# yjhuangcd/FI-ODE

Hardware: AMD Instinct MI355X
Metric: CIFAR-10 train-step images/sec (B=128, h_sample=256) at 1/2/4/8 MI355X (higher is better)
Workload: dtype f32; 1 GPU; hipGraph replay: BASELINE configs[1]: train step of README.md:27 at epoch 20 with train_ode (rk4, step_size 0.1, t_max=1: 10 steps / 40 train-mode f-evals, backprop through the stages; loss_ode portion 0.2) + the Lyapunov loss (B=128, h_sample_size=256 -> 204 uniform + 52 correct-cone rows/image), KWLarge-Cayley backbone + Adam; global_batch=128, h_sample_size=256, rows_per_rank=32768, parallelism=dp1

## Files before the change

fi-ode_amd/csrc/dense.hip:

```cpp
#include <hip/hip_runtime.h>
#include <stdint.h>

#include "common.h"
#include "fiode.h"

namespace {

constexpr int NT = 256;
constexpr int DPARTS = 256;

struct DArgs {
  int cout, cin, k, R, wide;
  const float* W;
  const float* alpha;
  const float* nrm;
};

__device__ __forceinline__ float wx(const DArgs& a, const float* Wb, int r, int c) {
  return a.wide ? Wb[(int64_t)c * a.cin + r] : Wb[(int64_t)r * a.cin + c];
}
__device__ __forceinline__ int64_t wpos(const DArgs& a, int r, int c) {
  return a.wide ? (int64_t)c * a.cin + r : (int64_t)r * a.cin + c;
}

// ... 134 lines not shown
  const float s = a.alpha[b] / a.nrm[b];
  const float* Wb = a.W + (int64_t)b * n;
  const float* P1b = P1 ? P1 + (int64_t)b * RV * k : nullptr;
  const float* P2b = P2 ? P2 + (int64_t)b * RV * k : nullptr;
  float* gXb = gX + (int64_t)b * n;
  float d = 0.f;
#pragma unroll 4
  for (int idx = blockIdx.x * NT + threadIdx.x; idx < n; idx += DPARTS * NT) {
    const int o = idx / a.cin, c = idx % a.cin;
    const int r = a.wide ? c : o;
    float g;
    if (r < k) {
      g = gXb[idx];
    } else {
      const int64_t pi = a.wide ? (int64_t)o * RV + (c - k) : (int64_t)(o - k) * k + c;
      g = s * P1b[pi] - 2.0f * P2b[pi];
      gXb[idx] = g;
    }
    d = fmaf(g, Wb[idx], d);
  }
  for (int o = 32; o > 0; o >>= 1) d += __shfl_xor(d, o);
  if ((threadIdx.x & 63) == 0) red[threadIdx.x >> 6] = d;
  __syncthreads();
  if (threadIdx.x == 0) {
    float t = 0.f;
    for (int q = 0; q < NT / 64; ++q) t += red[q];
    dpart[b * DPARTS + blockIdx.x] = t;
  }
}

__global__ void __launch_bounds__(NT) k_dense_gv4(DArgs a, const float* __restrict__ P1, const float* __restrict__ P2,
// ... 4 lines not shown
  const float* Wb = a.W + (int64_t)b * n;
  const float* P1b = P1 ? P1 + (int64_t)b * RV * k : nullptr;
  const float* P2b = P2 ? P2 + (int64_t)b * RV * k : nullptr;
  float* gXb = gX + (int64_t)b * n;
  float d = 0.f;
  for (int o = blockIdx.x; o < a.cout; o += DPARTS) {
    for (int c4 = threadIdx.x; c4 < c4n; c4 += NT) {
      const int c = 4 * c4;
      const int r = a.wide ? c : o;
      const int64_t idx = (int64_t)o * a.cin + c;
      f32x4 g;
      if (r < k) {
        g = *reinterpret_cast<const f32x4*>(gXb + idx);
      } else {
        const int64_t pi = a.wide ? (int64_t)o * RV + (c - k) : (int64_t)(o - k) * k + c;
        const f32x4 p1 = *reinterpret_cast<const f32x4*>(P1b + pi), p2 = *reinterpret_cast<const f32x4*>(P2b + pi);
#pragma unroll
        for (int e = 0; e < 4; ++e) g[e] = s * p1[e] - 2.0f * p2[e];
        *reinterpret_cast<f32x4*>(gXb + idx) = g;
      }
      const f32x4 w = *reinterpret_cast<const f32x4*>(Wb + idx);
#pragma unroll
      for (int e = 0; e < 4; ++e) d = fmaf(g[e], w[e], d);
    }
  }
  for (int o = 32; o > 0; o >>= 1) d += __shfl_xor(d, o);
  if ((threadIdx.x & 63) == 0) red[threadIdx.x >> 6] = d;
  __syncthreads();
  if (threadIdx.x == 0) {
    float t = 0.f;
    for (int q = 0; q < NT / 64; ++q) t += red[q];
    dpart[b * DPARTS + blockIdx.x] = t;
  }
// ... 78 lines not shown
      for (int x = 0; x < 2; ++x)
#pragma unroll
        for (int y = 0; y < 2; ++y)
          acc[x][y] = __builtin_amdgcn_mfma_f32_16x16x4f32(av[x][s], bv[y][s], acc[x][y], 0, 0, 0);
  }
#pragma unroll
  for (int x = 0; x < 2; ++x)
#pragma unroll
    for (int y = 0; y < 2; ++y)
#pragma unroll
      for (int r = 0; r < 4; ++r) red[w][16 * x + 4 * q + r][16 * y + i] = acc[x][y][r];
  __syncthreads();
  for (int e = threadIdx.x; e < 32 * 32; e += 256) {
    const int r = e >> 5, c = e & 31;
    C[(int64_t)(tm + r) * n + tn + c] = ((red[0][r][c] + red[1][r][c]) + red[2][r][c]) + red[3][r][c];
  }
}

int mk(const fiode_dense_config* cfg, DArgs& a, int& batch) {
  if (!cfg || cfg->batch < 1 || cfg->cout < 1 || cfg->cin < 1) return FIODE_EINVAL;
  a = DArgs{};
  a.cout = cfg->cout;
  a.cin = cfg->cin;
  a.wide = a.cin > a.cout;
  a.k = a.wide ? a.cout : a.cin;
  a.R = a.wide ? a.cin : a.cout;
  batch = cfg->batch;
  return FIODE_OK;
}

// ... 131 lines not shown
  a.nrm = nrm;
  hipStream_t st = (hipStream_t)stream;
  float* dpart = (float*)workspace;
  auto al16 = [](const void* q) { return ((uintptr_t)q & 15u) == 0; };
  const bool vec = a.cin % 4 == 0 && a.k % 4 == 0 && al16(W) && al16(gX) && al16(gW) && (!P1 || al16(P1)) &&
                   (!P2 || al16(P2));
  if (vec)
    hipLaunchKernelGGL(k_dense_gv4, dim3(DPARTS, batch), dim3(NT), 0, st, a, P1, P2, gX, dpart);
  else
    hipLaunchKernelGGL(k_dense_gv, dim3(DPARTS, batch), dim3(NT), 0, st, a, P1, P2, gX, dpart);
  hipLaunchKernelGGL(k_dense_gw, grid_for((int64_t)a.cout * a.cin, batch), dim3(NT), 0, st, a, (const float*)gX, dpart,
                     gW, galpha, vec ? 1 : 0);
  DENSE_RET();
}

extern "C" int fiode_dense_gemm(void* stream, int32_t batch, int32_t n, int32_t trans_a, int32_t trans_b,
                                const float* A, const float* B, float* C) {
  if (batch < 1 || batch > 65535 || n < 64 || !A || !B || !C) return FIODE_EINVAL;
  if (n % 64 != 0) return FIODE_ESHAPE;
  if ((((uintptr_t)A | (uintptr_t)B) & 15u) != 0) return FIODE_ESHAPE;
  const dim3 grid((unsigned)(n / 32), (unsigned)(n / 32), (unsigned)batch);
  hipStream_t st = (hipStream_t)stream;
  if (trans_a && trans_b) hipLaunchKernelGGL((k_dense_gemm<true, true>), grid, dim3(256), 0, st, n, A, B, C);
  else if (trans_a) hipLaunchKernelGGL((k_dense_gemm<true, false>), grid, dim3(256), 0, st, n, A, B, C);
  else if (trans_b) hipLaunchKernelGGL((k_dense_gemm<false, true>), grid, dim3(256), 0, st, n, A, B, C);
  else hipLaunchKernelGGL((k_dense_gemm<false, false>), grid, dim3(256), 0, st, n, A, B, C);
  DENSE_RET();
}
```

fi-ode_amd/fiode_amd/_lib.py:

```python
from __future__ import annotations

import ctypes as ct
import os
import pathlib

_HERE = pathlib.Path(__file__).resolve().parent
LIB_PATH = pathlib.Path(os.environ.get("FIODE_LIB", _HERE / "libfiode.so"))

FIODE_SAMPLER_GIVEN, FIODE_SAMPLER_COMPOSITE, FIODE_SAMPLER_DECISION_BOUNDARY, FIODE_SAMPLER_TRAJECTORY = 0, 1, 2, 3
FIODE_DROPOUT_OFF, FIODE_DROPOUT_GIVEN, FIODE_DROPOUT_PHILOX = 0, 1, 2
FIODE_ACT_RELU, FIODE_ACT_GROUPSORT = 0, 1

class FiodeLibraryError(RuntimeError):
    pass


class FiodeError(RuntimeError):
    pass


_fp = ct.POINTER(ct.c_float)
_vp = ct.c_void_p


# ... 171 lines not shown
        "fiode_dense_cayley_prep": (ct.c_int, [_vp, ct.POINTER(DenseConfig), _vp, _vp, _vp, _vp, _vp]),
        "fiode_dense_norm_workspace_bytes": (ct.c_size_t, [ct.POINTER(DenseConfig)]),
        "fiode_dense_norm_partials": (ct.c_int, [_vp, ct.POINTER(DenseConfig), _vp, _vp, ct.c_size_t]),
        "fiode_dense_cayley_prep_normed": (ct.c_int, [_vp, ct.POINTER(DenseConfig), _vp, _vp, _vp, _vp, _vp, _vp]),
        "fiode_dense_norm_partials_clear": (ct.c_int, [_vp, ct.POINTER(DenseConfig), _vp, _vp, ct.c_size_t, _vp,
                                                       ct.c_size_t, ct.c_size_t]),
        "fiode_dense_inverse_flag_bytes": (ct.c_size_t, [ct.c_int32]),
        "fiode_dense_cayley_inverse": (ct.c_int, [_vp, ct.POINTER(DenseConfig), _vp, _vp, _vp, _vp, _vp, _vp, _vp,
                                                  _vp, ct.c_size_t]),
        "fiode_dense_cayley_finish": (ct.c_int, [_vp, ct.POINTER(DenseConfig), _vp, _vp, _vp, _vp, _vp]),
        "fiode_dense_cayley_ginv": (ct.c_int, [_vp, ct.POINTER(DenseConfig), _vp, _vp, _vp, _vp, _vp]),
        "fiode_dense_cayley_h": (ct.c_int, [_vp, ct.POINTER(DenseConfig), _vp, _vp, _vp]),
        "fiode_dense_cayley_workspace_bytes": (ct.c_size_t, [ct.POINTER(DenseConfig)]),
        "fiode_dense_cayley_grad": (ct.c_int, [_vp, ct.POINTER(DenseConfig), _vp, _vp, _vp, _vp, _vp, _vp, _vp, _vp,
                                               _vp, ct.c_size_t]),
        "fiode_dense_gemm": (ct.c_int, [_vp, ct.c_int32, ct.c_int32, ct.c_int32, ct.c_int32, _vp, _vp, _vp]),
        "fiode_gemm_splits": (ct.c_int32, [ct.POINTER(GemmDesc)]),
        "fiode_gemm_counter_bytes": (ct.c_size_t, [ct.POINTER(GemmDesc)]),
        "fiode_gemm_workspace_bytes": (ct.c_size_t, [ct.POINTER(GemmDesc)]),
        "fiode_gemm": (ct.c_int, [_vp, ct.POINTER(GemmDesc), _vp, _vp, _vp, _vp, _vp, ct.c_size_t]),
        "fiode_gemm_pair_workspace_bytes": (ct.c_size_t, [ct.POINTER(GemmDesc), ct.POINTER(GemmDesc)]),
        "fiode_gemm_pair": (ct.c_int, [_vp, ct.POINTER(GemmDesc), _vp, _vp, _vp, _vp, ct.POINTER(GemmDesc), _vp, _vp,
                                       _vp, _vp, _vp, ct.c_size_t]),
        "fiode_sconv_rfft2": (ct.c_int, [_vp, ct.POINTER(SconvConfig), _vp, _vp, _vp, _vp]),
        "fiode_sconv_irfft2": (ct.c_int, [_vp, ct.POINTER(SconvConfig), _vp, _vp, ct.c_int32, _vp, _vp]),
        "fiode_sconv_rfft2_nchw": (ct.c_int, [_vp, ct.POINTER(SconvConfig), _vp, _vp, _vp, _vp]),
        "fiode_sconv_irfft2_qx": (ct.c_int, [_vp, ct.POINTER(SconvConfig), _vp, _vp, ct.c_int32, _vp, ct.c_int32,
                                             _vp, _vp]),
        "fiode_cgemm": (ct.c_int, [_vp, ct.c_int32, ct.c_int32, ct.c_int32, ct.c_int32, ct.c_int32, ct.c_int32, _vp,
                                   _vp, _vp, _vp]),
# ... 40 lines not shown
```

fi-ode_amd/fiode_amd/cayley.py:

```python
from __future__ import annotations

import ctypes as ct
import math
from typing import Optional

import torch
import torch.nn as nn
import torch.nn.functional as F

from .streams import current, fork, join, prefetch, run_on, shared, take


_BLOCK = 128


def _block_inverse(M: torch.Tensor) -> torch.Tensor:
    from . import ops
    n = M.shape[-1]
    if n > 64 and M.dtype == torch.float32 and M.is_cuda:
        if M.dim() == 2:
            return ops.block_inverse(M)
        return ops.block_inverse(M.reshape(-1, n, n)).reshape(M.shape)
    if n <= _BLOCK:
        return ops.batched_inverse(M)
# ... 172 lines not shown
                     device=Wb.device)
    L.check(lib.fiode_dense_cayley_grad(st, ct.byref(cfg), Wb.data_ptr(), al.data_ptr(), nrm.data_ptr(),
                                        ops._ptr(P1), ops._ptr(P2), gX.data_ptr(), gW.data_ptr(), ga.data_ptr(),
                                        ws.data_ptr(), ws.numel()), "fiode_dense_cayley_grad")
    return gW.reshape(wshape), ga.reshape(ashape)


def _dense_fused_ok(W: torch.Tensor) -> bool:
    from . import _lib as L
    k = min(W.shape[-2], W.shape[-1])
    lib = L.lib()
    return (DENSE_FUSED_INVERSE and W.is_cuda and hasattr(lib, "fiode_dense_cayley_inverse")
            and lib.fiode_dense_inverse_flag_bytes(k) > 0)


def _dense_forward_fused(W: torch.Tensor, alpha: torch.Tensor):
    from . import ops, _lib as L
    Wb = W.detach().reshape(-1, W.shape[-2], W.shape[-1]).contiguous()
    al = alpha.detach().reshape(-1).contiguous().float()
    b, cout, cin = Wb.shape
    wide = cin > cout
    k = cout if wide else cin
    cfg = L.DenseConfig(b, cout, cin)
    lib, stream = L.lib(), ops._stream(W.device)
    per = lib.fiode_block_inverse_workspace_bytes(k)
    ws = ops._Workspace.get(W.device, b * per, f"denseinv{torch.cuda.current_stream(W.device).cuda_stream}")
    part = torch.empty(lib.fiode_dense_norm_workspace_bytes(ct.byref(cfg)) // 4, dtype=torch.float32, device=W.device)
    L.check(lib.fiode_dense_norm_partials_clear(stream, ct.byref(cfg), Wb.data_ptr(), part.data_ptr(), part.numel() * 4,
                                                ws.data_ptr(), lib.fiode_dense_inverse_flag_bytes(k) // 4, per),
            "fiode_dense_norm_partials_clear")
    Vp = (Wb[:, :, k:].mT if wide else Wb[:, k:, :]) if max(cout, cin) > k else None
    G = ops.mm(Vp.mT, Vp, site="dense_fwd") if Vp is not None else None
    nrm = torch.empty(b, dtype=torch.float32, device=W.device)
    inv = torch.empty((b, k, k), dtype=torch.float32, device=W.device)
    Q = torch.empty_like(Wb) if Vp is None else None
    L.check(lib.fiode_dense_cayley_inverse(stream, ct.byref(cfg), Wb.data_ptr(), al.data_ptr(), part.data_ptr(),
                                           ops._ptr(G), nrm.data_ptr(), inv.data_ptr(), ops._ptr(Q), ws.data_ptr(),
                                           ws.numel()), "fiode_dense_cayley_inverse")
    st = dict(Wb=Wb, al=al, nrm=nrm, wide=wide, k=k, Vp=Vp, cfg=cfg)
    if Q is None:
        Q = _dense_finish(st, inv)
    return st, inv, Q


class _DenseCayleyFn(torch.autograd.Function):

    @staticmethod
    def forward(ctx, W, alpha):
        if _dense_fused_ok(W):
            st, inv, Q = _dense_forward_fused(W, alpha)
        else:
            st, M = _dense_prep(W, alpha)
            inv = _block_inverse(M)
            Q = _dense_finish(st, inv)
        ctx.save_for_backward(st["Wb"], st["al"], st["nrm"], inv)
# ... 78 lines not shown
        return top
    return torch.cat([top, -2.0 * (V @ inv)], dim=-2)


DENSE_GEMM = True
DENSE_NORM_PARTIALS = True


class CayleyLinear(nn.Linear):

    def __init__(self, in_features: int, out_features: int, bias: bool = True):
        super().__init__(in_features, out_features, bias)
        self.alpha = nn.Parameter(self.weight.detach().norm().reshape(1).clone())
        self._Q = None
        self._pre = None

    def reset_parameters(self) -> None:
        std = 1.0 / math.sqrt(self.weight.shape[1])
        nn.init.uniform_(self.weight, -std, std)
        if self.bias is not None:
            nn.init.uniform_(self.bias, -std, std)
        self._Q = None

    def effective_weight(self) -> torch.Tensor:
        return cayley_scaled(self.weight, self.alpha)

    def prefetch(self, stream: torch.cuda.Stream) -> None:
        self._pre = prefetch(stream, self.effective_weight)

    def forward_weight_unjoined(self):
        if self._pre is not None and self.training:
            (Q, ev), self._pre = self._pre, None
            Q.record_stream(torch.cuda.current_stream(Q.device))
            self._Q = Q.detach()
            return Q, ev
        return self.forward_weight(), None

    def forward_weight(self) -> torch.Tensor:
        if self._pre is not None and self.training:
            Q = take(self._pre)
            self._pre = None
        elif self.training or self._Q is None:
            Q = self.effective_weight()
        else:
            Q = self._Q
        self._Q = Q.detach()
        return Q if self.training else self._Q

    def forward(self, x: torch.Tensor) -> torch.Tensor:
        return F.linear(x, self.forward_weight(), self.bias)


HEAD_WGRAD_SIDE = True
# ... 31 lines not shown
        g = g.contiguous()

        def wgrad(k, gk, x):
            return fork(_head_stream(g.device, k), lambda: (ops.mm(gk.t(), x, site="head"), gk.sum(0)), reads=(gk, x))

        w3 = wgrad(3, g, z2)
        g2 = ops.head_out_backward_gs(g, Q3, y2) if ctx.out_k else ops.groupsort_backward(y2, ops.mm(g, Q3, site="head"), 1)
        w2 = wgrad(2, g2, z1)
        g1 = ops.groupsort_backward(y1, ops.mm(g2, Q2, site="head"), 1)
        w1 = wgrad(1, g1, h)
        dh = ops.mm(g1, Q1, site="head")
        (dW3, db3), (dW2, db2), (dW1, db1) = join(w3, w2, w1)
        return dh, dW1, db1, dW2, db2, dW3, db3, None


HEAD_OUT_KERNEL = True
HEAD_OUT_MAX_J = 16


def _head_out_ok(Q3: torch.Tensor) -> bool:
    return HEAD_OUT_KERNEL and Q3.shape[0] <= HEAD_OUT_MAX_J


def linear_head(mods, h: torch.Tensor):
    fusable = (HEAD_WGRAD_SIDE and h.is_cuda and len(mods) == 5 and
               all(isinstance(m, CayleyLinear) and m.training and m.bias is not None for m in mods[0::2]) and
               all(isinstance(m, GroupSort) for m in mods[1::2]) and torch.is_grad_enabled())
    if not fusable:
        for m in mods:
            h = m(h)
        return h
    l1, l2, l3 = mods[0::2]
    Q1 = l1.forward_weight()
    (Q2, j2), (Q3, j3) = l2.forward_weight_unjoined(), l3.forward_weight_unjoined()
    return _LinearHeadFn.apply(h.contiguous(), Q1, l1.bias, Q2, l2.bias, Q3, l3.bias, (j2, j3))


class _GroupSortFn(torch.autograd.Function):
    @staticmethod
    def forward(ctx, x, cdim: int):
        from . import ops
        y = ops.groupsort_forward(x, cdim)
        ctx.save_for_backward(x)
        ctx.cdim = cdim
        return y

    @staticmethod
# ... 263 lines not shown
```

fi-ode_amd/fiode_amd/checkpoint.py:

```python
from __future__ import annotations

import os
from typing import Any, Dict, Iterable, Optional, Tuple

import torch
from torch import nn

LIGHTNING_VERSION = "1.6.0"


class CheckpointError(RuntimeError):
    pass


def read_checkpoint(path: str | os.PathLike, map_location: Any = "cpu") -> Dict[str, Any]:
    try:
        ck = torch.load(path, map_location=map_location, weights_only=True)
    except Exception as e:
        raise CheckpointError(f"cannot read {path} with torch.load(weights_only=True): {e}") from e
    if not isinstance(ck, dict):
        raise CheckpointError(f"{path}: expected a dict checkpoint, got {type(ck).__name__}")
    return ck


# ... 4 lines not shown
        raise CheckpointError(f"non-tensor entries in the state_dict: {bad[:5]}")
    return sd


def load_state(module: nn.Module, state_dict: Dict[str, torch.Tensor], strict: bool = False
               ) -> Tuple[list, list]:
    own = module.state_dict()
    shape_bad = [(k, tuple(v.shape), tuple(own[k].shape)) for k, v in state_dict.items()
                 if k in own and tuple(own[k].shape) != tuple(v.shape)]
    if shape_bad:
        raise CheckpointError("shape mismatch (key, checkpoint, module): " + "; ".join(map(str, shape_bad[:5])))
    res = module.load_state_dict(state_dict, strict=strict)
    for m in module.modules():
        if getattr(m, "_pre", None) is not None:
            m._pre = None
    return list(res.missing_keys), list(res.unexpected_keys)


def load_from_checkpoint(module: nn.Module, path: str | os.PathLike, strict: bool = False,
                         map_location: Any = None) -> Dict[str, Any]:
    ck = read_checkpoint(path, map_location="cpu" if map_location is None else map_location)
    sd = checkpoint_state_dict(ck)
    missing, unexpected = load_state(module, sd, strict=strict)
    return dict(missing_keys=missing, unexpected_keys=unexpected, epoch=ck.get("epoch"),
                global_step=ck.get("global_step"))


def save_checkpoint(module: nn.Module, path: str | os.PathLike, epoch: int = 0, global_step: int = 0,
                    optimizers: Optional[Iterable[torch.optim.Optimizer]] = None,
                    extra: Optional[Dict[str, Any]] = None) -> None:
# ... 40 lines not shown
```

fi-ode_amd/fiode_amd/models.py:

```python
from __future__ import annotations

from typing import Optional, Sequence

import torch
import torch.nn as nn

from .cayley import CayleyConv, CayleyLinear, GroupSort, linear_head


class Normalize(nn.Module):

    def __init__(self, mu: Sequence[float], std: Optional[Sequence[float]]):
        super().__init__()
        self.register_buffer("mu", torch.tensor(list(mu), dtype=torch.float32).view(-1, 1, 1))
        self.register_buffer("std", None if std is None else torch.tensor(list(std), dtype=torch.float32).view(-1, 1, 1))

    fused_hwcb = True

    def forward(self, x):
        if self.fused_hwcb and x.is_cuda and x.dtype == torch.float32 and x.dim() == 4 and not x.requires_grad:
            from . import _lib as L, ops
            B, C, H, W = x.shape
            xc = x.contiguous()
            y = torch.empty((H, W, C, B), dtype=torch.float32, device=x.device)
# ... 15 lines not shown
        act_fn = GroupSort if act == "GroupSort" else nn.ReLU
        self.model = nn.Sequential(
            CayleyConv(3, 32 * w, 3), act_fn(),
            CayleyConv(32 * w, 32 * w, 3, stride=2), act_fn(),
            CayleyConv(32 * w, 64 * w, 3), act_fn(),
            CayleyConv(64 * w, 64 * w, 3, stride=2), act_fn(),
            nn.Flatten(),
            CayleyLinear(4096 * w, 512 * w), act_fn(),
            CayleyLinear(512 * w, 512), act_fn(),
            CayleyLinear(512, out_dim),
        )

        self.spatial_major = True
        self.fused_transforms = True
        self.nchw_last = True

    def can_take_nchw(self, x) -> bool:
        m = self.model[0]
        return (self.spatial_major and self.fused_transforms and x.is_cuda and x.dtype == torch.float32
                and x.dim() == 4 and not x.requires_grad and isinstance(m, CayleyConv) and not m.downsample
                and x.shape[-1] == x.shape[-2] and x.shape[-1] in (8, 16, 32))

    def forward(self, x, norm=None):
        if not (self.spatial_major and x.is_cuda):
            return self.model(x)
        mods = list(self.model)
        i = 0
        nconv = 0
        if norm is not None:
            if getattr(self, "after_conv_hook", None) is not None:
                self.after_conv_hook(-1)
            gs = isinstance(mods[1], GroupSort)
            h = mods[0].forward_nchw_fused(x, norm[0], norm[1], gs)
            i = 2 if gs else 1
            if getattr(self, "after_conv_hook", None) is not None:
                self.after_conv_hook(0)
            nconv = 1
        else:
            h = x.permute(2, 3, 1, 0).contiguous()
            if getattr(self, "after_conv_hook", None) is not None:
                self.after_conv_hook(-1)
# ... 8 lines not shown
                    i += 2 if gs else 1
                    if getattr(self, "after_conv_hook", None) is not None:
                        self.after_conv_hook(nconv)
                    nconv += 1
                    continue
                h = m.forward_hwcb(h)
                if getattr(self, "after_conv_hook", None) is not None:
                    self.after_conv_hook(nconv)
                nconv += 1
            elif isinstance(m, GroupSort):
                h = m(h, channel_dim=2)
            else:
                h = m(h)
            i += 1
        h = h.reshape(h.shape[0], -1) if nchw else h.permute(3, 2, 0, 1).reshape(h.shape[3], -1)
        return linear_head(mods[i + 1:], h)


class NormalizedBackbone(nn.Sequential):

    fused_input = True

    def forward(self, x):
        norm, net = self[0], self[1]
        if (self.fused_input and len(self) == 2 and isinstance(norm, Normalize) and isinstance(net, KWLargeConcat)
                and norm.fused_hwcb and net.can_take_nchw(x)):
            return net(x.contiguous(), norm=(norm.mu, norm.std))
        return super().forward(x)


def make_ortho_KWLarge_Concat(n_in_channels=3, n_outputs=10, mu=(0.485, 0.456, 0.406), std=(0.225, 0.225, 0.225),
# ... 47 lines not shown
```

fi-ode_amd/fiode_amd/ops.py:

```python
from __future__ import annotations

import ctypes as ct
from dataclasses import dataclass
from typing import Dict, Optional

import torch

from . import _lib as L

C, M, X = 10, 128, 10
WEIGHT_KEYS = ("Q1", "b1", "Qx", "bx", "Q2", "b2", "Q3", "b3")
WEIGHT_SHAPES = {"Q1": (M, C), "b1": (M,), "Qx": (M, X), "bx": (M,), "Q2": (M, M), "b2": (M,),
                 "Q3": (C, M), "b3": (C,)}


@dataclass
class DynCfg:
    alpha_1: float = 100.0
    alpha_2: float = 20.0
    sigma_1: float = 0.02
    scale_nominal: bool = True
    dropout: float = 0.5
    qp_max_iter: int = 30
    qp_tol: float = 1e-4
# ... 690 lines not shown
                                _ptr(scale), A.data_ptr(), B.data_ptr(), C.data_ptr()), "fiode_cgemm")
    return C


def _mat_layout(X: torch.Tensor):
    R, Cn = X.shape[-2], X.shape[-1]
    s0, s1 = X.stride(-2), X.stride(-1)
    if (s1 == 1 or Cn == 1) and (s0 >= Cn or R == 1):
        return 0, max(s0 if R > 1 else Cn, Cn, 1)
    if (s0 == 1 or R == 1) and (s1 >= R or Cn == 1):
        return 1, max(s1 if Cn > 1 else R, R, 1)
    return None


MM_LIBRARY = False
MM_LIBRARY_SITES: set = {"dense_fwd", "dense_bwd", "head"}
MM_PAIR = True


def _gemm_ws(dev: torch.device, nbytes: int) -> torch.Tensor:
    return _Workspace.get(dev, nbytes, f"gemm{torch.cuda.current_stream(dev).cuda_stream}", zero=True)


def _gemm_operands(A: torch.Tensor, B: torch.Tensor, alpha: float, beta: float, bias, out, split_k: int,
                   max_workgroups: int):
    dev = B.device
    if A.dtype != torch.float32 or B.dtype != torch.float32 or A.device != dev or dev.type != "cuda":
        raise ValueError(f"mm: float32 ROCm operands, got {A.dtype} on {A.device}, {B.dtype} on {B.device}")
    if A.dim() not in (2, 3) or B.dim() not in (2, 3) or A.shape[-1] != B.shape[-2]:
        raise ValueError(f"mm: shapes {tuple(A.shape)} @ {tuple(B.shape)}")
    batch = max(A.shape[0] if A.dim() == 3 else 1, B.shape[0] if B.dim() == 3 else 1)
# ... 27 lines not shown
                   float(alpha), float(beta), int(split_k), int(max_workgroups))
    return d, A, B, bias, out


def mm(A: torch.Tensor, B: torch.Tensor, *, alpha: float = 1.0, beta: float = 0.0,
       bias: Optional[torch.Tensor] = None, out: Optional[torch.Tensor] = None, split_k: int = 0,
       max_workgroups: int = 0, site: str = "") -> torch.Tensor:
    dev = B.device
    if MM_LIBRARY or site in MM_LIBRARY_SITES:
        if out is None and alpha == 1.0 and beta == 0.0:
            if bias is not None and A.dim() == 2 and B.dim() == 2:
                return torch.addmm(bias, A, B)
            r = torch.matmul(A, B)
            return (r + bias if bias is not None else r).contiguous()
        d, A, B, bias, out = _gemm_operands(A, B, alpha, beta, bias, out, split_k, max_workgroups)
        r = torch.matmul(A, B)
        r = r * alpha if alpha != 1.0 else r
        if bias is not None:
            r = r + bias
        if beta != 0.0:
            r = r + beta * out
        out.copy_(r)
        return out
    d, A, B, bias, out = _gemm_operands(A, B, alpha, beta, bias, out, split_k, max_workgroups)
    lib = L.lib()
    nb = lib.fiode_gemm_workspace_bytes(ct.byref(d))
    ws = _gemm_ws(dev, nb) if nb else None
    L.check(lib.fiode_gemm(_stream(dev), ct.byref(d), A.data_ptr(), B.data_ptr(), _ptr(bias), out.data_ptr(),
                           _ptr(ws), ws.numel() if ws is not None else 0), "fiode_gemm")
    return out
# ... 134 lines not shown
```

include/fiode.h:

```cpp
#ifndef FIODE_H_
#define FIODE_H_

#include <stddef.h>
#include <stdint.h>

#ifdef __cplusplus
extern "C" {
#endif

#define FIODE_ABI_VERSION 5

#if defined(__GNUC__)
#define FIODE_API __attribute__((visibility("default")))
#else
#define FIODE_API
#endif

enum {
  FIODE_OK = 0,
  FIODE_EINVAL = 1,
  FIODE_ESHAPE = 2,
  FIODE_EWORKSPACE = 3,
  FIODE_EHIP = 100
};
// ... 241 lines not shown
                                              void* workspace, size_t workspace_bytes, void* clear,
                                              size_t clear_words, size_t clear_stride_bytes);
FIODE_API size_t fiode_dense_inverse_flag_bytes(int32_t k);
FIODE_API int fiode_dense_cayley_inverse(void* stream, const fiode_dense_config* cfg, const float* W,
                                         const float* alpha, const float* part, const float* G, float* nrm_out,
                                         float* inv_out, float* q_out, void* workspace, size_t workspace_bytes);
FIODE_API int fiode_dense_cayley_finish(void* stream, const fiode_dense_config* cfg, const float* alpha,
                                        const float* nrm, const float* inv, const float* P, float* Q);
FIODE_API int fiode_dense_cayley_ginv(void* stream, const fiode_dense_config* cfg, const float* alpha,
                                      const float* nrm, const float* gQ, const float* A, float* Ginv);
FIODE_API int fiode_dense_cayley_h(void* stream, const fiode_dense_config* cfg, const float* GMn, float* gX, float* H);
FIODE_API size_t fiode_dense_cayley_workspace_bytes(const fiode_dense_config* cfg);
FIODE_API int fiode_dense_cayley_grad(void* stream, const fiode_dense_config* cfg, const float* W, const float* alpha,
                                      const float* nrm, const float* P1, const float* P2, float* gX, float* gW,
                                      float* galpha, void* workspace, size_t workspace_bytes);
FIODE_API int fiode_dense_gemm(void* stream, int32_t batch, int32_t n, int32_t trans_a, int32_t trans_b,
                               const float* A, const float* B, float* C);

typedef struct fiode_gemm_desc {
  int32_t batch, M, N, K;
  int32_t trans_a, trans_b;
  int64_t lda, ldb, ldc;
  int64_t stride_a, stride_b, stride_c;
  float alpha, beta;
  int32_t split_k;
  int32_t max_workgroups;
} fiode_gemm_desc;
FIODE_API int32_t fiode_gemm_splits(const fiode_gemm_desc* d);
FIODE_API size_t fiode_gemm_counter_bytes(const fiode_gemm_desc* d);
FIODE_API size_t fiode_gemm_workspace_bytes(const fiode_gemm_desc* d);
// ... 75 lines not shown
```

Baseline: 106,400 images/s.

## Apply first Cayley head layer in factored form instead of materializing Q

For the wide first linear layer of the head, the Cayley-orthogonal weight Q is no longer built explicitly. The head applies the inverse directly to the batch (h minus scaled T, times inv) using new skinny MFMA kernels, with matching input-grad and symmetric pair kernels for the backward pass and a merged weight-gradient path. This skips the O(k^2·cin) finish GEMM and its backward, in exchange for extra per-batch GEMMs, new autograd plumbing and side-stream joins. It also routes plain 2D library matmuls straight to torch.mm/addmm.

```diff
diff --git a/fi-ode_amd/csrc/dense.hip b/fi-ode_amd/csrc/dense.hip
--- a/fi-ode_amd/csrc/dense.hip
+++ b/fi-ode_amd/csrc/dense.hip
@@ -172,7 +172,7 @@
       g = gXb[idx];
     } else {
       const int64_t pi = a.wide ? (int64_t)o * RV + (c - k) : (int64_t)(o - k) * k + c;
-      g = s * P1b[pi] - 2.0f * P2b[pi];
+      g = P2b ? s * P1b[pi] - 2.0f * P2b[pi] : P1b[pi];
       gXb[idx] = g;
     }
     d = fmaf(g, Wb[idx], d);
@@ -207,9 +207,14 @@
         g = *reinterpret_cast<const f32x4*>(gXb + idx);
       } else {
         const int64_t pi = a.wide ? (int64_t)o * RV + (c - k) : (int64_t)(o - k) * k + c;
-        const f32x4 p1 = *reinterpret_cast<const f32x4*>(P1b + pi), p2 = *reinterpret_cast<const f32x4*>(P2b + pi);
-#pragma unroll
-        for (int e = 0; e < 4; ++e) g[e] = s * p1[e] - 2.0f * p2[e];
+        const f32x4 p1 = *reinterpret_cast<const f32x4*>(P1b + pi);
+        if (P2b) {
+          const f32x4 p2 = *reinterpret_cast<const f32x4*>(P2b + pi);
+#pragma unroll
+          for (int e = 0; e < 4; ++e) g[e] = s * p1[e] - 2.0f * p2[e];
+        } else {
+          g = p1;
+        }
         *reinterpret_cast<f32x4*>(gXb + idx) = g;
       }
       const f32x4 w = *reinterpret_cast<const f32x4*>(Wb + idx);
@@ -318,6 +323,169 @@
   for (int e = threadIdx.x; e < 32 * 32; e += 256) {
     const int r = e >> 5, c = e & 31;
     C[(int64_t)(tm + r) * n + tn + c] = ((red[0][r][c] + red[1][r][c]) + red[2][r][c]) + red[3][r][c];
+  }
+}
+
+template <int NW, int UNR, class LA, class LB>
+__device__ __forceinline__ void skinny_wave(int K, int w, int q, LA load_a, LB load_b, f32x4 (&acc)[2][2]) {
+#pragma unroll
+  for (int x = 0; x < 2; ++x)
+#pragma unroll
+    for (int y = 0; y < 2; ++y) acc[x][y] = f32x4{0.f, 0.f, 0.f, 0.f};
+  for (int c0 = 16 * w; c0 < K; c0 += 16 * NW * UNR) {
+    f32x4 av[UNR][2], bv[UNR][2];
+#pragma unroll
+    for (int u = 0; u < UNR; ++u) {
+      const int c = c0 + 16 * NW * u, kb = c + 4 * q;
+#pragma unroll
+      for (int x = 0; x < 2; ++x) av[u][x] = c < K ? load_a(x, kb) : f32x4{0.f, 0.f, 0.f, 0.f};
+#pragma unroll
+      for (int y = 0; y < 2; ++y) bv[u][y] = c < K ? load_b(y, kb) : f32x4{0.f, 0.f, 0.f, 0.f};
+    }
+#pragma unroll
+    for (int u = 0; u < UNR; ++u)
+#pragma unroll
+      for (int s = 0; s < 4; ++s)
+#pragma unroll
+        for (int x = 0; x < 2; ++x)
+#pragma unroll
+          for (int y = 0; y < 2; ++y)
+            acc[x][y] = __builtin_amdgcn_mfma_f32_16x16x4f32(av[u][x][s], bv[u][y][s], acc[x][y], 0, 0, 0);
+  }
+}
+
+template <int NW>
+__device__ __forceinline__ void skinny_store(float (&red)[NW][32][33], int w, int i, int q, const f32x4 (&acc)[2][2]) {
+#pragma unroll
+  for (int x = 0; x < 2; ++x)
+#pragma unroll
+    for (int y = 0; y < 2; ++y)
+#pragma unroll
+      for (int r = 0; r < 4; ++r) red[w][16 * x + 4 * q + r][16 * y + i] = acc[x][y][r];
+}
+
+template <int NW>
+__device__ __forceinline__ float skinny_sum(const float (&red)[NW][32][33], int r, int c) {
+  float v = red[0][r][c];
+#pragma unroll
+  for (int w = 1; w < NW; ++w) v += red[w][r][c];
+  return v;
+}
+
+constexpr int HEAD_NW = 8;
+
+__global__ void __launch_bounds__(64 * HEAD_NW) k_head_apply(int B, int k, int ldh, const float* __restrict__ alpha,
+                                                    const float* __restrict__ nrm, const float* __restrict__ h,
+                                                    const float* __restrict__ T, const float* __restrict__ inv,
+                                                    const float* __restrict__ bias, float* __restrict__ Y,
+                                                    float* __restrict__ y1) {
+  __shared__ float red[HEAD_NW][32][33];
+  const int lane = threadIdx.x & 63, w = threadIdx.x >> 6, i = lane & 15, q = lane >> 4;
+  const int tm = blockIdx.y * 32, tn = blockIdx.x * 32;
+  const float s = alpha[0] / nrm[0];
+  f32x4 acc[2][2];
+  skinny_wave<HEAD_NW, 4>(
+      k, w, q,
+      [&](int x, int kb) {
+        const int m = tm + 16 * x + i;
+        f32x4 e = f32x4{0.f, 0.f, 0.f, 0.f};
+        if (m < B) {
+          const f32x4 hu = *reinterpret_cast<const f32x4*>(h + (int64_t)m * ldh + kb);
+          const f32x4 t = *reinterpret_cast<const f32x4*>(T + (int64_t)m * k + kb);
+#pragma unroll
+          for (int u = 0; u < 4; ++u) e[u] = hu[u] - s * t[u];
+        }
+        return e;
+      },
+      [&](int y, int kb) {
+        const int c = tn + 16 * y + i;
+        f32x4 b;
+#pragma unroll
+        for (int u = 0; u < 4; ++u) b[u] = inv[(int64_t)(kb + u) * k + c];
+        return b;
+      },
+      acc);
+  skinny_store(red, w, i, q, acc);
+  __syncthreads();
+  for (int e = threadIdx.x; e < 32 * 32; e += 64 * HEAD_NW) {
+    const int r = e >> 5, c = e & 31, m = tm + r, n = tn + c;
+    if (m >= B) continue;
+    const float v = skinny_sum(red, r, c);
+    Y[(int64_t)m * k + n] = v;
+    y1[(int64_t)m * k + n] = (2.0f * v - h[(int64_t)m * ldh + n]) + (bias ? bias[n] : 0.f);
+  }
+}
+
+__global__ void __launch_bounds__(64 * HEAD_NW) k_head_input_grad(int B, int k, int lddh, const float* __restrict__ alpha,
+                                                         const float* __restrict__ nrm, const float* __restrict__ g,
+                                                         const float* __restrict__ inv, float* __restrict__ dh,
+                                                         float* __restrict__ Zn, float* __restrict__ Z2) {
+  __shared__ float red[HEAD_NW][32][33];
+  const int lane = threadIdx.x & 63, w = threadIdx.x >> 6, i = lane & 15, q = lane >> 4;
+  const int tm = blockIdx.y * 32, tn = blockIdx.x * 32;
+  const float s = alpha[0] / nrm[0];
+  f32x4 acc[2][2];
+  skinny_wave<HEAD_NW, 4>(
+      k, w, q,
+      [&](int x, int kb) {
+        const int m = tm + 16 * x + i;
+        return m < B ? *reinterpret_cast<const f32x4*>(g + (int64_t)m * k + kb) : f32x4{0.f, 0.f, 0.f, 0.f};
+      },
+      [&](int y, int kb) { return *reinterpret_cast<const f32x4*>(inv + (int64_t)(tn + 16 * y + i) * k + kb); },
+      acc);
+  skinny_store(red, w, i, q, acc);
+  __syncthreads();
+  for (int e = threadIdx.x; e < 32 * 32; e += 64 * HEAD_NW) {
+    const int r = e >> 5, c = e & 31, m = tm + r, n = tn + c;
+    if (m >= B) continue;
+    const float z = skinny_sum(red, r, c), zn = -2.0f * z;
+    dh[(int64_t)m * lddh + n] = 2.0f * z - g[(int64_t)m * k + n];
+    Zn[(int64_t)m * k + n] = zn;
+    Z2[(int64_t)m * k + n] = s * zn;
+  }
+}
+
+__global__ void __launch_bounds__(256) k_head_sym_pair(int B, int k, int cin, const float* __restrict__ alpha,
+                                                       const float* __restrict__ nrm, const float* __restrict__ Y,
+                                                       const float* __restrict__ Zn, float* __restrict__ gX,
+                                                       float* __restrict__ Hs) {
+  __shared__ float redp[4][32][33];
+  __shared__ float redr[4][32][33];
+  const int lane = threadIdx.x & 63, w = threadIdx.x >> 6, i = lane & 15, q = lane >> 4;
+  const int nt = k >> 5;
+  int ti = 0, rem = blockIdx.x;
+  while (rem >= nt - ti) {
+    rem -= nt - ti;
+    ++ti;
+  }
+  const int tj = ti + rem;
+  const float s = alpha[0] / nrm[0];
+  auto col4 = [&](const float* __restrict__ X, int c, int kb) {
+    f32x4 v;
+#pragma unroll
+    for (int u = 0; u < 4; ++u) v[u] = kb + u < B ? X[(int64_t)(kb + u) * k + c] : 0.f;
+    return v;
+  };
+  f32x4 acc[2][2];
+  skinny_wave<4, 2>(
+      B, w, q, [&](int x, int kb) { return col4(Y, 32 * ti + 16 * x + i, kb); },
+      [&](int y, int kb) { return col4(Zn, 32 * tj + 16 * y + i, kb); }, acc);
+  skinny_store(redp, w, i, q, acc);
+  skinny_wave<4, 2>(
+      B, w, q, [&](int x, int kb) { return col4(Y, 32 * tj + 16 * x + i, kb); },
+      [&](int y, int kb) { return col4(Zn, 32 * ti + 16 * y + i, kb); }, acc);
+  skinny_store(redr, w, i, q, acc);
+  __syncthreads();
+  for (int e = threadIdx.x; e < 32 * 32; e += 256) {
+    const int a = e >> 5, b = e & 31;
+    if (ti == tj && a > b) continue;
+    const int I = 32 * ti + a, J = 32 * tj + b;
+    const float gij = skinny_sum(redp, a, b), gji = skinny_sum(redr, b, a);
+    const float hv = s * (gij + gji), u = gij - gji;
+    Hs[(int64_t)I * k + J] = hv;
+    Hs[(int64_t)J * k + I] = hv;
+    gX[(int64_t)J * cin + I] = u;
+    gX[(int64_t)I * cin + J] = -u;
   }
 }
 
@@ -479,6 +647,76 @@
   DENSE_RET();
 }
 
+extern "C" int fiode_dense_cayley_grad_merged(void* stream, const fiode_dense_config* cfg, const float* W,
+                                              const float* alpha, const float* nrm, const float* P1m, float* gX,
+                                              float* gW, float* galpha, void* workspace, size_t workspace_bytes) {
+  DArgs a;
+  int batch, rc = mk(cfg, a, batch);
+  if (rc) return rc;
+  if (!W || !alpha || !nrm || !gX || !gW || !galpha || !workspace || (a.R > a.k && !P1m)) return FIODE_EINVAL;
+  if (workspace_bytes < fiode_dense_cayley_workspace_bytes(cfg)) return FIODE_EWORKSPACE;
+  a.W = W;
+  a.alpha = alpha;
+  a.nrm = nrm;
+  hipStream_t st = (hipStream_t)stream;
+  float* dpart = (float*)workspace;
+  auto al16 = [](const void* q) { return ((uintptr_t)q & 15u) == 0; };
+  const bool vec = a.cin % 4 == 0 && a.k % 4 == 0 && al16(W) && al16(gX) && al16(gW) && (!P1m || al16(P1m));
+  if (vec)
+    hipLaunchKernelGGL(k_dense_gv4, dim3(DPARTS, batch), dim3(NT), 0, st, a, P1m, (const float*)nullptr, gX, dpart);
+  else
+    hipLaunchKernelGGL(k_dense_gv, dim3(DPARTS, batch), dim3(NT), 0, st, a, P1m, (const float*)nullptr, gX, dpart);
+  hipLaunchKernelGGL(k_dense_gw, grid_for((int64_t)a.cout * a.cin, batch), dim3(NT), 0, st, a, (const float*)gX, dpart,
+                     gW, galpha, vec ? 1 : 0);
+  DENSE_RET();
+}
+
+namespace {
+int head_shape(const fiode_dense_config* cfg, int32_t rows) {
+  if (!cfg || cfg->batch != 1 || cfg->cout < 1 || cfg->cin < 1 || rows < 1) return FIODE_EINVAL;
+  if (cfg->cin <= cfg->cout || cfg->cout % 64 != 0 || cfg->cin % 4 != 0 || rows > 32 * 65535) return FIODE_ESHAPE;
+  return FIODE_OK;
+}
+bool al16(const void* q) { return ((uintptr_t)q & 15u) == 0; }
+}
+
+extern "C" int fiode_head_apply(void* stream, const fiode_dense_config* cfg, int32_t rows, const float* alpha,
+                                const float* nrm, const float* h, const float* T, const float* inv,
+                                const float* bias, float* Y, float* y1) {
+  const int rc = head_shape(cfg, rows);
+  if (rc) return rc;
+  if (!alpha || !nrm || !h || !T || !inv || !Y || !y1) return FIODE_EINVAL;
+  if (!al16(h) || !al16(T)) return FIODE_ESHAPE;
+  const int k = cfg->cout;
+  hipLaunchKernelGGL(k_head_apply, dim3(k / 32, (rows + 31) / 32), dim3(64 * HEAD_NW), 0, (hipStream_t)stream, (int)rows, k,
+                     (int)cfg->cin, alpha, nrm, h, T, inv, bias, Y, y1);
+  DENSE_RET();
+}
+
+extern "C" int fiode_head_input_grad(void* stream, const fiode_dense_config* cfg, int32_t rows, const float* alpha,
+                                     const float* nrm, const float* g, const float* inv, float* dh, float* Zn,
+                                     float* Z2) {
+  const int rc = head_shape(cfg, rows);
+  if (rc) return rc;
+  if (!alpha || !nrm || !g || !inv || !dh || !Zn || !Z2) return FIODE_EINVAL;
+  if (!al16(g) || !al16(inv)) return FIODE_ESHAPE;
+  const int k = cfg->cout;
+  hipLaunchKernelGGL(k_head_input_grad, dim3(k / 32, (rows + 31) / 32), dim3(64 * HEAD_NW), 0, (hipStream_t)stream, (int)rows,
+                     k, (int)cfg->cin, alpha, nrm, g, inv, dh, Zn, Z2);
+  DENSE_RET();
+}
+
+extern "C" int fiode_head_sym_pair(void* stream, const fiode_dense_config* cfg, int32_t rows, const float* alpha,
+                                   const float* nrm, const float* Y, const float* Zn, float* gX, float* Hs) {
+  const int rc = head_shape(cfg, rows);
+  if (rc) return rc;
+  if (!alpha || !nrm || !Y || !Zn || !gX || !Hs) return FIODE_EINVAL;
+  const int k = cfg->cout, nt = k / 32;
+  hipLaunchKernelGGL(k_head_sym_pair, dim3(nt * (nt + 1) / 2), dim3(256), 0, (hipStream_t)stream, (int)rows, k,
+                     (int)cfg->cin, alpha, nrm, Y, Zn, gX, Hs);
+  DENSE_RET();
+}
+
 extern "C" int fiode_dense_gemm(void* stream, int32_t batch, int32_t n, int32_t trans_a, int32_t trans_b,
                                 const float* A, const float* B, float* C) {
   if (batch < 1 || batch > 65535 || n < 64 || !A || !B || !C) return FIODE_EINVAL;
diff --git a/fi-ode_amd/fiode_amd/_lib.py b/fi-ode_amd/fiode_amd/_lib.py
--- a/fi-ode_amd/fiode_amd/_lib.py
+++ b/fi-ode_amd/fiode_amd/_lib.py
@@ -209,6 +209,13 @@
         "fiode_dense_cayley_workspace_bytes": (ct.c_size_t, [ct.POINTER(DenseConfig)]),
         "fiode_dense_cayley_grad": (ct.c_int, [_vp, ct.POINTER(DenseConfig), _vp, _vp, _vp, _vp, _vp, _vp, _vp, _vp,
                                                _vp, ct.c_size_t]),
+        "fiode_dense_cayley_grad_merged": (ct.c_int, [_vp, ct.POINTER(DenseConfig), _vp, _vp, _vp, _vp, _vp, _vp, _vp,
+                                                      _vp, ct.c_size_t]),
+        "fiode_head_apply": (ct.c_int, [_vp, ct.POINTER(DenseConfig), ct.c_int32, _vp, _vp, _vp, _vp, _vp, _vp, _vp,
+                                        _vp]),
+        "fiode_head_input_grad": (ct.c_int, [_vp, ct.POINTER(DenseConfig), ct.c_int32, _vp, _vp, _vp, _vp, _vp, _vp,
+                                             _vp]),
+        "fiode_head_sym_pair": (ct.c_int, [_vp, ct.POINTER(DenseConfig), ct.c_int32, _vp, _vp, _vp, _vp, _vp, _vp]),
         "fiode_dense_gemm": (ct.c_int, [_vp, ct.c_int32, ct.c_int32, ct.c_int32, ct.c_int32, _vp, _vp, _vp]),
         "fiode_gemm_splits": (ct.c_int32, [ct.POINTER(GemmDesc)]),
         "fiode_gemm_counter_bytes": (ct.c_size_t, [ct.POINTER(GemmDesc)]),
diff --git a/fi-ode_amd/fiode_amd/cayley.py b/fi-ode_amd/fiode_amd/cayley.py
--- a/fi-ode_amd/fiode_amd/cayley.py
+++ b/fi-ode_amd/fiode_amd/cayley.py
@@ -210,7 +210,7 @@
             and lib.fiode_dense_inverse_flag_bytes(k) > 0)
 
 
-def _dense_forward_fused(W: torch.Tensor, alpha: torch.Tensor):
+def _dense_forward_fused(W: torch.Tensor, alpha: torch.Tensor, finish: bool = True):
     from . import ops, _lib as L
     Wb = W.detach().reshape(-1, W.shape[-2], W.shape[-1]).contiguous()
     al = alpha.detach().reshape(-1).contiguous().float()
@@ -234,7 +234,7 @@
                                            ops._ptr(G), nrm.data_ptr(), inv.data_ptr(), ops._ptr(Q), ws.data_ptr(),
                                            ws.numel()), "fiode_dense_cayley_inverse")
     st = dict(Wb=Wb, al=al, nrm=nrm, wide=wide, k=k, Vp=Vp, cfg=cfg)
-    if Q is None:
+    if Q is None and finish:
         Q = _dense_finish(st, inv)
     return st, inv, Q
 
@@ -343,6 +343,8 @@
         self.alpha = nn.Parameter(self.weight.detach().norm().reshape(1).clone())
         self._Q = None
         self._pre = None
+        self.factored = False
+        self._pre_f = None
 
     def reset_parameters(self) -> None:
         std = 1.0 / math.sqrt(self.weight.shape[1])
@@ -355,7 +357,15 @@
         return cayley_scaled(self.weight, self.alpha)
 
     def prefetch(self, stream: torch.cuda.Stream) -> None:
-        self._pre = prefetch(stream, self.effective_weight)
+        if self.factored and _factored_ok(self):
+            self._pre, self._pre_f = None, prefetch(stream, self._factored_state)
+            return
+        self._pre, self._pre_f = prefetch(stream, self.effective_weight), None
+
+    def _factored_state(self):
+        box = {}
+        inv = _FactoredMapFn.apply(self.weight, self.alpha, box)
+        return box["st"], inv, box
 
     def forward_weight_unjoined(self):
         if self._pre is not None and self.training:
@@ -366,6 +376,7 @@
         return self.forward_weight(), None
 
     def forward_weight(self) -> torch.Tensor:
+        self._pre_f = None
         if self._pre is not None and self.training:
             Q = take(self._pre)
             self._pre = None
@@ -427,6 +438,129 @@
         return dh, dW1, db1, dW2, db2, dW3, db3, None
 
 
+def _factored_ok(l1: "CayleyLinear", h: Optional[torch.Tensor] = None) -> bool:
+    W = l1.weight
+    return (FACTORED_HEAD and DENSE_FUSED and W.dim() == 2 and W.dtype == torch.float32 and W.is_cuda
+            and W.shape[1] > W.shape[0] and W.shape[1] % 4 == 0 and l1.training and torch.is_grad_enabled()
+            and _dense_fused_ok(W) and (h is None or (h.is_cuda and h.dtype == torch.float32)))
+
+
+FACTORED_HEAD = True
+
+
+def _factored_apply(h, Wd, b1, pre):
+    from . import ops, _lib as L
+    B, k = h.shape[0], Wd.shape[0]
+    Tp = ops.mm(h[:, k:], Wd[:, k:].t(), site="head_t")
+    st, inv = take(pre)
+    b1 = b1.contiguous()
+    Y, y1 = torch.empty_like(Tp), torch.empty_like(Tp)
+    L.check(L.lib().fiode_head_apply(ops._stream(h.device), ct.byref(st["cfg"]), B, st["al"].data_ptr(),
+                                     st["nrm"].data_ptr(), h.data_ptr(), Tp.data_ptr(), inv.data_ptr(),
+                                     b1.data_ptr(), Y.data_ptr(), y1.data_ptr()), "fiode_head_apply")
+    return Y, y1, st, inv
+
+
+def _factored_dh_u(cfg, al, nrm, inv, g1, h):
+    from . import ops, _lib as L
+    dh = torch.empty_like(h)
+    Zn, Z2 = torch.empty_like(g1), torch.empty_like(g1)
+    L.check(L.lib().fiode_head_input_grad(ops._stream(h.device), ct.byref(cfg), h.shape[0], al.data_ptr(),
+                                          nrm.data_ptr(), g1.data_ptr(), inv.data_ptr(), dh.data_ptr(), Zn.data_ptr(),
+                                          Z2.data_ptr()), "fiode_head_input_grad")
+    return dh, Zn, Z2
+
+
+def _factored_wgrad(cfg, Wd, al, nrm, Y, Zn, h):
+    from . import ops, _lib as L
+    lib, st, dev, k = L.lib(), ops._stream(h.device), h.device, Wd.shape[0]
+    gX = torch.empty_like(Wd)
+    Hs = torch.empty((k, k), dtype=torch.float32, device=dev)
+    L.check(lib.fiode_head_sym_pair(st, ct.byref(cfg), h.shape[0], al.data_ptr(), nrm.data_ptr(), Y.data_ptr(),
+                                    Zn.data_ptr(), gX.data_ptr(), Hs.data_ptr()), "fiode_head_sym_pair")
+    P1m = ops.mm(Hs, Wd[:, k:], site="head_gv")
+    ops.mm(Zn.t(), h[:, k:], beta=1.0, out=P1m, site="head_gv")
+    gW = torch.empty_like(Wd)
+    ga = torch.empty(1, dtype=torch.float32, device=dev)
+    ws = torch.empty(max(1, lib.fiode_dense_cayley_workspace_bytes(ct.byref(cfg))), dtype=torch.uint8, device=dev)
+    L.check(lib.fiode_dense_cayley_grad_merged(st, ct.byref(cfg), Wd.data_ptr(), al.data_ptr(), nrm.data_ptr(),
+                                               P1m.data_ptr(), gX.data_ptr(), gW.data_ptr(), ga.data_ptr(),
+                                               ws.data_ptr(), ws.numel()), "fiode_dense_cayley_grad_merged")
+    return gW, ga
+
+
+def _factored_bias_grad(g1):
+    return g1.sum(0)
+
+
+class _FactoredMapFn(torch.autograd.Function):
+
+    @staticmethod
+    def forward(ctx, W, alpha, box):
+        st, inv, _ = _dense_forward_fused(W, alpha, finish=False)
+        box["st"] = st
+        ctx.box, ctx.shapes = box, (W.shape, alpha.shape)
+        return inv
+
+    @staticmethod
+    def backward(ctx, _token):
+        branch = ctx.box.pop("wgrad", None)
+        if branch is None:
+            raise RuntimeError("_FactoredMapFn: the inverse of a factored layer is differentiated only through "
+                               "_FactoredHeadFn")
+        (gW, ga), = join(branch)
+        return gW.reshape(ctx.shapes[0]), ga.reshape(ctx.shapes[1]), None
+
+
+class _FactoredHeadFn(torch.autograd.Function):
+
+    @staticmethod
+    def forward(ctx, h, inv, b1, Q2, b2, Q3, b3, st, box, ev, joins=None):
+        from . import ops
+        j2, j3 = joins if joins is not None else (None, None)
+        cur = torch.cuda.current_stream(h.device)
+        Wd = st["Wb"][0]
+        Y, y1, _, inv = _factored_apply(h, Wd, b1.detach(), ((st, inv), ev))
+        z1 = ops.groupsort_forward(y1, 1)
+        if j2 is not None:
+            cur.wait_event(j2)
+        y2 = ops.mm(z1, Q2.t(), bias=b2, site="head")
+        z2 = ops.groupsort_forward(y2, 1)
+        if j3 is not None:
+            cur.wait_event(j3)
+        out_k = _head_out_ok(Q3)
+        out = ops.head_out(z2, Q3, b3) if out_k else ops.mm(z2, Q3.t(), bias=b3, site="head")
+        ctx.save_for_backward(h, Wd, st["al"], st["nrm"], inv, Y, Q2, Q3, y1, z1, y2, z2)
+        ctx.out_k, ctx.cfg, ctx.box = out_k, st["cfg"], box
+        return out
+
+    @staticmethod
+    def backward(ctx, g):
+        from . import ops
+        h, Wd, al, nrm, inv, Y, Q2, Q3, y1, z1, y2, z2 = ctx.saved_tensors
+        cfg = ctx.cfg
+        g = g.contiguous()
+        dev, k = g.device, Wd.shape[0]
+
+        def wgrad(i, gk, x):
+            return fork(_head_stream(dev, i), lambda: (ops.mm(gk.t(), x, site="head"), gk.sum(0)), reads=(gk, x))
+
+        w3 = wgrad(3, g, z2)
+        g2 = ops.head_out_backward_gs(g, Q3, y2) if ctx.out_k else ops.groupsort_backward(y2, ops.mm(g, Q3, site="head"), 1)
+        w2 = wgrad(2, g2, z1)
+        g1 = ops.groupsort_backward(y1, ops.mm(g2, Q2, site="head"), 1).contiguous()
+        wb = fork(_head_stream(dev, 2), lambda: _factored_bias_grad(g1), reads=(g1,))
+        dh, Zn, Z2 = _factored_dh_u(cfg, al, nrm, inv, g1, h)
+        ops.mm(Z2, Wd[:, k:], out=dh[:, k:], site="head_dhv")
+        token = None
+        if ctx.needs_input_grad[1]:
+            ctx.box["wgrad"] = fork(_head_stream(dev, 1), lambda: _factored_wgrad(cfg, Wd, al, nrm, Y, Zn, h),
+                                    reads=(Zn, Y, h, inv, nrm))
+            token = inv
+        (dW3, db3), (dW2, db2), db1 = join(w3, w2, wb)
+        return dh, token, db1, dW2, db2, dW3, db3, None, None, None, None
+
+
 HEAD_OUT_KERNEL = True
 HEAD_OUT_MAX_J = 16
 
@@ -435,7 +569,7 @@
     return HEAD_OUT_KERNEL and Q3.shape[0] <= HEAD_OUT_MAX_J
 
 
-def linear_head(mods, h: torch.Tensor):
+def linear_head(mods, h: torch.Tensor, factored: bool = False):
     fusable = (HEAD_WGRAD_SIDE and h.is_cuda and len(mods) == 5 and
                all(isinstance(m, CayleyLinear) and m.training and m.bias is not None for m in mods[0::2]) and
                all(isinstance(m, GroupSort) for m in mods[1::2]) and torch.is_grad_enabled())
@@ -444,6 +578,12 @@
             h = m(h)
         return h
     l1, l2, l3 = mods[0::2]
+    if factored and l1._pre is None and _factored_ok(l1, h):
+        pre, l1._pre_f = l1._pre_f, None
+        (st, inv, box), ev = pre if pre is not None else (l1._factored_state(), None)
+        l1._Q = None
+        (Q2, j2), (Q3, j3) = l2.forward_weight_unjoined(), l3.forward_weight_unjoined()
+        return _FactoredHeadFn.apply(h.contiguous(), inv, l1.bias, Q2, l2.bias, Q3, l3.bias, st, box, ev, (j2, j3))
     Q1 = l1.forward_weight()
     (Q2, j2), (Q3, j3) = l2.forward_weight_unjoined(), l3.forward_weight_unjoined()
     return _LinearHeadFn.apply(h.contiguous(), Q1, l1.bias, Q2, l2.bias, Q3, l3.bias, (j2, j3))
diff --git a/fi-ode_amd/fiode_amd/checkpoint.py b/fi-ode_amd/fiode_amd/checkpoint.py
--- a/fi-ode_amd/fiode_amd/checkpoint.py
+++ b/fi-ode_amd/fiode_amd/checkpoint.py
@@ -42,6 +42,8 @@
     for m in module.modules():
         if getattr(m, "_pre", None) is not None:
             m._pre = None
+        if getattr(m, "_pre_f", None) is not None:
+            m._pre_f = None
     return list(res.missing_keys), list(res.unexpected_keys)
 
 
diff --git a/fi-ode_amd/fiode_amd/models.py b/fi-ode_amd/fiode_amd/models.py
--- a/fi-ode_amd/fiode_amd/models.py
+++ b/fi-ode_amd/fiode_amd/models.py
@@ -53,6 +53,7 @@
         self.spatial_major = True
         self.fused_transforms = True
         self.nchw_last = True
+        self.factored_head = True
 
     def can_take_nchw(self, x) -> bool:
         m = self.model[0]
@@ -64,6 +65,9 @@
         if not (self.spatial_major and x.is_cuda):
             return self.model(x)
         mods = list(self.model)
+        for j, m in enumerate(mods):
+            if isinstance(m, nn.Flatten) and j + 1 < len(mods) and isinstance(mods[j + 1], CayleyLinear):
+                mods[j + 1].factored = bool(self.factored_head)
         i = 0
         nconv = 0
         if norm is not None:
@@ -102,7 +106,7 @@
                 h = m(h)
             i += 1
         h = h.reshape(h.shape[0], -1) if nchw else h.permute(3, 2, 0, 1).reshape(h.shape[3], -1)
-        return linear_head(mods[i + 1:], h)
+        return linear_head(mods[i + 1:], h, factored=bool(self.factored_head))
 
 
 class NormalizedBackbone(nn.Sequential):
diff --git a/fi-ode_amd/fiode_amd/ops.py b/fi-ode_amd/fiode_amd/ops.py
--- a/fi-ode_amd/fiode_amd/ops.py
+++ b/fi-ode_amd/fiode_amd/ops.py
@@ -728,7 +728,7 @@
 
 
 MM_LIBRARY = False
-MM_LIBRARY_SITES: set = {"dense_fwd", "dense_bwd", "head"}
+MM_LIBRARY_SITES: set = {"dense_fwd", "dense_bwd", "head", "head_t", "head_dhv", "head_gv"}
 MM_PAIR = True
 
 
@@ -786,6 +786,8 @@
             r = torch.matmul(A, B)
             return (r + bias if bias is not None else r).contiguous()
         d, A, B, bias, out = _gemm_operands(A, B, alpha, beta, bias, out, split_k, max_workgroups)
+        if A.dim() == 2 and B.dim() == 2 and alpha == 1.0 and bias is None and beta in (0.0, 1.0):
+            return torch.mm(A, B, out=out) if beta == 0.0 else out.addmm_(A, B)
         r = torch.matmul(A, B)
         r = r * alpha if alpha != 1.0 else r
         if bias is not None:
diff --git a/include/fiode.h b/include/fiode.h
--- a/include/fiode.h
+++ b/include/fiode.h
@@ -279,6 +279,17 @@
 FIODE_API int fiode_dense_cayley_grad(void* stream, const fiode_dense_config* cfg, const float* W, const float* alpha,
                                       const float* nrm, const float* P1, const float* P2, float* gX, float* gW,
                                       float* galpha, void* workspace, size_t workspace_bytes);
+FIODE_API int fiode_dense_cayley_grad_merged(void* stream, const fiode_dense_config* cfg, const float* W,
+                                             const float* alpha, const float* nrm, const float* P1m, float* gX,
+                                             float* gW, float* galpha, void* workspace, size_t workspace_bytes);
+FIODE_API int fiode_head_apply(void* stream, const fiode_dense_config* cfg, int32_t rows, const float* alpha,
+                               const float* nrm, const float* h, const float* T, const float* inv,
+                               const float* bias, float* Y, float* y1);
+FIODE_API int fiode_head_input_grad(void* stream, const fiode_dense_config* cfg, int32_t rows, const float* alpha,
+                                    const float* nrm, const float* g, const float* inv, float* dh, float* Zn,
+                                    float* Z2);
+FIODE_API int fiode_head_sym_pair(void* stream, const fiode_dense_config* cfg, int32_t rows, const float* alpha,
+                                  const float* nrm, const float* Y, const float* Zn, float* gX, float* Hs);
 FIODE_API int fiode_dense_gemm(void* stream, int32_t batch, int32_t n, int32_t trans_a, int32_t trans_b,
                                const float* A, const float* B, float* C);
 
```

Result: no change. 108,600 images/s (median of 5 runs) (+2.1%).
